# jinhan/tacotron2-vae

Measured on AMD Instinct MI355X. Metric: mel-frames/s (train step, batch=6, 80-mel), higher is better.
Workload: dtype f32; 1 GPU; configs[1]: Tacotron2-VAE fp32 train step (fwd+loss+bwd+clip+Adam), B=6/GPU fixed shape T_in=84 T_out=400, dropout on, random-init seed 1234; step_mode=hip-graph replay, decoder_forward=persistent, decoder_backward=persistent, startup_steps=43, global_batch=6, parallelism=dp1

## Files before the change

### include/t2vae.h

```cpp
#ifndef T2VAE_H
#define T2VAE_H
#include <stdint.h>
#ifdef __cplusplus
extern "C" {
#endif

#define T2V_OK 0
#define T2V_ERR_DIMS -1
#define T2V_ERR_ARG -2
#define T2V_ERR_LAUNCH -3

const char* t2v_version(void);
const char* t2v_last_error(void);

void t2v_set_phase_profile(unsigned long long* dev_buf32);
int t2v_stamp(unsigned long long* dev_buf, int slot, void* stream);
int t2v_debug_spin(int wgs, int microseconds, void* stream);

typedef struct t2v_step_params {
    uint64_t epoch;
    float lr;
    float bc1;
    float bc2s;
    float kl_weight;
// ... 210 lines not shown

int t2v_bn_act_fwd(const float* y, const float* stat_part, int nblk, const float* gamma, const float* beta,
                   float* running_mean, float* running_var, float* mean_out, float* rstd_out, float* out,
                   int B, int M, int T, int act, int training, float p_drop, float momentum, float eps,
                   uint64_t seed, uint32_t rng_stream, uint32_t rng_t, void* stream);
int t2v_bn_act_fwd_len(const float* y, const float* gamma, const float* beta, const float* running_mean,
                       const float* running_var, float* out, const int32_t* lengths, int B, int M, int T, int act, float eps,
                       void* stream);
int t2v_bn_act_bwd(const float* y, const float* dout, const float* mean, const float* rstd,
                   const float* gamma, const float* beta, float* dy, float* dgamma, float* dbeta,
                   float* dconv_bias, int B, int M, int T, int act, float p_drop, uint64_t seed,
                   uint32_t rng_stream, uint32_t rng_t, void* stream);
int t2v_bn_act_bwd_eval(const float* y, const float* dout, const float* mean, const float* rstd,
                   const float* gamma, const float* beta, float* dy, float* dgamma, float* dbeta,
                   float* dconv_bias, int B, int M, int T, int act, float p_drop, uint64_t seed,
                   uint32_t rng_stream, uint32_t rng_t, void* stream);

int t2v_embedding_fwd(const long long* ids, const float* W, float* out_bct, int B, int T, int C, int n_symbols, void* stream);
int t2v_embedding_bwd(const long long* ids, const float* dy_bct, float* dW, int B, int T, int C, int n_symbols, void* stream);

int t2v_gemm_epilogue_bwd(const float* dy, const float* y, float* out, size_t n, float scale, void* stream);

long t2v_colsum_scratch_floats(long M, long N);
int t2v_colsum(const float* A, long lda, long M, long N, float* scratch, float* out, void* stream);

int t2v_mask_outputs(float* mel, float* mel_post, float* gate, const int* lengths, int B, int C, int T, float gate_fill,
                     void* stream);
int t2v_mask_time(const float* x, float* out, const int32_t* lengths, int B, int C, int T, void* stream);
int t2v_reparam_fwd(const float* eps, const float* mu, const float* logvar, float* z, long n, void* stream);
int t2v_reparam_bwd(const float* dz, const float* eps, const float* logvar, float* dlogvar, long n, void* stream);
int t2v_gather_words(const void* const* src, void* const* dst, int n, void* stream);
int t2v_concat2_rows(const float* a, long lda, int na, const float* b, long ldb, int nb, float* out, long rows, void* stream);

int t2v_bilstm_fwd(const float* gx, const float* whh, const int32_t* lengths, float* y, float* gates,
                   float* cells, float* hx_scratch, uint32_t* sync3, int B, int T, void* stream);
int t2v_bilstm_bwd(const float* whh, const int32_t* lengths, const float* dy, const float* gates,
                   const float* cells, float* dg, float* dgx_scratch, uint32_t* sync3, int B, int T,
                   void* stream);

int t2v_gemm_f32(const float* A, long sAi, long sAk, const float* B, long sBj, long sBk, const float* bias,
                 float* C, int ldc, int M, int N, int K, int relu, int accumulate, float p_drop,
                 uint64_t seed, uint32_t rng_stream, uint32_t rng_t, void* stream);
long t2v_gemm_splitk_scratch_floats(int M, int N, int K);
int t2v_gemm_f32_splitk(const float* A, long sAi, long sAk, const float* B, long sBj, long sBk, const float* bias,
                        float* C, int ldc, int M, int N, int K, int relu, int accumulate, float p_drop,
                        uint64_t seed, uint32_t rng_stream, uint32_t rng_t, float* splitk_scratch, void* stream);

int t2v_gemm_f32_set_mode(int x3);

typedef struct t2v_gemm_group {
    const float* A;
    long sAi;
    long sAk;
    int nb;
    const float* B[3];
    long sBj[3];
    long sBk[3];
    int N[3];
    float* C[3];
    int ldc[3];
} t2v_gemm_group;
long t2v_gemm_f32_grouped_scratch_floats(const t2v_gemm_group* groups, int ngroups, int M, int K);
int t2v_gemm_f32_grouped(const t2v_gemm_group* groups, int ngroups, int M, int K, int accumulate, float* scratch, void* stream);
long t2v_gemm_f32_grouped_group_offset(const t2v_gemm_group* groups, int ngroups, int M, int K, int g);
int t2v_gemm_f32_grouped_handed(const t2v_gemm_group* groups, int ngroups, int M, int K, int accumulate, float* scratch, int handed,
                                const uint32_t* done_ctr, int done_cap, void* stream);
long t2v_gemm_bf16_grouped_scratch_floats(const t2v_gemm_group* groups, int ngroups, int M, int K);
int t2v_gemm_bf16_grouped(const t2v_gemm_group* groups, int ngroups, int M, int K, int accumulate, float* scratch, void* stream);
// ... 111 lines not shown
```

### tacotron2-vae_amd/csrc/bilstm.hip

```cpp
#include "t2v_common.h"
#include "t2v_kernels.h"
#include "t2v_coop.h"

#define BL_H 256
#define BL_G (4 * BL_H)
#define BL_NW 16
#define BL_UNITS (BL_H / BL_NW)
#define BL_NT (BL_UNITS / 16)

struct BiLstmFwdArgs {
    const float* gx;
    const float* whh;
    const int32_t* lengths;
    float* y;
    float* gates;
    float* cells;
    t2v_u64* hx;
    unsigned* sync;
    int B, T;
};

#define BL_SPIN 4000000u
__device__ __forceinline__ void bl_put(t2v_u64* p, float v, unsigned tag) {
    __hip_atomic_store(p, ((t2v_u64)tag << 32) | (t2v_u64)__float_as_uint(v), __ATOMIC_RELAXED, __HIP_MEMORY_SCOPE_AGENT);
}

template <int BQ>
__global__ __launch_bounds__(512) void k_bilstm_fwd(BiLstmFwdArgs a) {
    const int dir = blockIdx.x / BL_NW, j = blockIdx.x % BL_NW;
    const int tid = threadIdx.x, wave = (tid >> 6) & 3, kh = tid >> 8, lane = tid & 63;
    const int b = lane & 15, g = lane >> 4;
    const bool bvalid = b < a.B;
    __shared__ float hbuf[16][BL_H + 4];
    __shared__ f32x4 kpart[4][BL_NT][64];
    __shared__ int ok_flag;
    if (tid == 0) ok_flag = 1;
    float wreg[BL_NT][32];
    {
        const float* W = a.whh + (size_t)dir * BL_G * BL_H;
#pragma unroll
        for (int tt = 0; tt < BL_NT; ++tt) {
            const int unit = j * BL_UNITS + (BL_NT * wave + tt) * 4 + ((lane & 15) >> 2);
            const int row = (lane & 3) * BL_H + unit;
#pragma unroll
            for (int s = 0; s < 32; ++s) wreg[tt][s] = W[(size_t)row * BL_H + 4 * (32 * kh + s) + g];
        }
    }
    for (int i = tid; i < 16 * (BL_H + 4); i += 512) (&hbuf[0][0])[i] = 0.f;
    const int len = bvalid ? a.lengths[b] : 0;
    float cst[BL_NT];
#pragma unroll
    for (int tt = 0; tt < BL_NT; ++tt) cst[tt] = 0.f;
    __syncthreads();

    for (int step = 0; step < a.T; ++step) {
        const bool active = step < len;
        const int t = dir == 0 ? step : len - 1 - step;
        float gxv[BL_NT][4];
#pragma unroll
        for (int tt = 0; tt < BL_NT; ++tt) {
            const int U = j * BL_UNITS + (BL_NT * wave + tt) * 4 + g;
#pragma unroll
            for (int r = 0; r < 4; ++r)
                gxv[tt][r] = (active && kh == 0) ? a.gx[(((size_t)dir * a.B + b) * a.T + t) * BL_G + r * BL_H + U] : 0.f;
        }
        f32x4 accv[BL_NT];
#pragma unroll
        for (int tt = 0; tt < BL_NT; ++tt) accv[tt] = f32x4{0.f, 0.f, 0.f, 0.f};
        const float* hrow = &hbuf[b][g + 128 * kh];
#pragma unroll
        for (int s = 0; s < 32; ++s) {
            const float hv = hrow[4 * s];
#pragma unroll
            for (int tt = 0; tt < BL_NT; ++tt) accv[tt] = mfma16x4(wreg[tt][s], hv, accv[tt]);
        }
        if (kh == 1) {
#pragma unroll
            for (int tt = 0; tt < BL_NT; ++tt) kpart[wave][tt][lane] = accv[tt];
        }
        __syncthreads();
        if (kh == 0) {
#pragma unroll
            for (int tt = 0; tt < BL_NT; ++tt) accv[tt] += kpart[wave][tt][lane];
        }
        t2v_u64* hx_w = a.hx + ((size_t)(dir * 2 + (step & 1)) * 16) * BL_H;
#pragma unroll
        for (int tt = 0; tt < BL_NT; ++tt) {
            const f32x4 acc = accv[tt];
            const int U = j * BL_UNITS + (BL_NT * wave + tt) * 4 + g;
            if (bvalid && kh == 0) {
                float hnew = hbuf[b][U];
                float gi = 0.f, gf = 0.f, gg = 0.f, go = 0.f, c = 0.f;
                if (active) {
                    gi = sigmoidf_(acc[0] + gxv[tt][0]); gf = sigmoidf_(acc[1] + gxv[tt][1]);
                    gg = tanhf_(acc[2] + gxv[tt][2]); go = sigmoidf_(acc[3] + gxv[tt][3]);
                    c = gf * cst[tt] + gi * gg;
                    cst[tt] = c;
                    hnew = go * tanhf_(c);
                }
                bl_put(hx_w + (size_t)b * BL_H + U, hnew, (unsigned)step + 1u);
                if (active) {
                    a.y[((size_t)b * a.T + t) * (2 * BL_H) + dir * BL_H + U] = hnew;
                    if (a.gates) {
                        float* gs = a.gates + (((size_t)dir * a.B + b) * a.T + t) * BL_G + U;
                        gs[0] = gi; gs[BL_H] = gf; gs[2 * BL_H] = gg; gs[3 * BL_H] = go;
                        a.cells[(((size_t)dir * a.B + b) * a.T + t) * BL_H + U] = c;
                    }
                }
            }
        }
        if (step + 1 == a.T) break;
        {
            float hv[BQ];
            unsigned spins = 0;
            for (; tid < BL_H;) {
                bool ok = true;
#pragma unroll
                for (int u = 0; u < BQ; ++u) {
                    const t2v_u64 x = __hip_atomic_load(hx_w + (size_t)min(u, a.B - 1) * BL_H + tid, __ATOMIC_RELAXED, __HIP_MEMORY_SCOPE_AGENT);
                    hv[u] = __uint_as_float((unsigned)x);
                    ok = ok && (unsigned)(x >> 32) == (unsigned)step + 1u;
                }
                if (ok) break;
                __builtin_amdgcn_s_sleep(1);
                if (++spins > BL_SPIN || __hip_atomic_load(a.sync + 2, __ATOMIC_RELAXED, __HIP_MEMORY_SCOPE_AGENT)) {
                    __hip_atomic_store(a.sync + 2, 1u, __ATOMIC_RELAXED, __HIP_MEMORY_SCOPE_AGENT);
                    ok_flag = 0;
                    break;
                }
            }
            __syncthreads();
#pragma unroll
            for (int u = 0; u < BQ; ++u)
                if (u < a.B && tid < BL_H) hbuf[u][tid] = hv[u];
        }
        __syncthreads();
        if (!ok_flag) return;
    }
}

struct BiLstmBwdArgs {
    const float* whh;
    const int32_t* lengths;
    const float* dy;
    const float* gates;
    const float* cells;
    float* dg;
    t2v_u64* dgx;
    unsigned* sync;
    int B, T;
};

#define BLB_GR ((size_t)16 * 16 * BL_H)
__global__ __launch_bounds__(512) void k_bilstm_bwd(BiLstmBwdArgs a) {
    const int dir = blockIdx.x / BL_NW, j = blockIdx.x % BL_NW;
    const int tid = threadIdx.x, wave = tid >> 6, lane = tid & 63;
    const int b = lane & 15, g = lane >> 4;
    __shared__ __attribute__((aligned(16))) float dgl[16][64 + 4];
    __shared__ int ok_flag;
    if (tid == 0) ok_flag = 1;
    float wreg[2][16];
    {
        const float* W = a.whh + (size_t)dir * BL_G * BL_H;
#pragma unroll
        for (int s = 0; s < 16; ++s) {
            const int k = 4 * s + g;
            const int row = (k >> 4) * BL_H + j * BL_UNITS + (k & 15);
// ... 68 lines not shown
        }
        if (live) { dgl[bb][uu] = di; dgl[bb][16 + uu] = df; dgl[bb][32 + uu] = dgg; dgl[bb][48 + uu] = dob; }
        __syncthreads();
        if (!ok_flag) return;
        if (step == 0) break;
        {
            float bop[16];
#pragma unroll
            for (int s = 0; s < 16; ++s) bop[s] = dgl[b][4 * s + g];
            __builtin_amdgcn_sched_barrier(0);
            f32x4 acc[2];
#pragma unroll
            for (int tt = 0; tt < 2; ++tt) acc[tt] = f32x4{0.f, 0.f, 0.f, 0.f};
#pragma unroll
            for (int s = 0; s < 16; ++s)
#pragma unroll
                for (int tt = 0; tt < 2; ++tt) acc[tt] = mfma16x4(wreg[tt][s], bop[s], acc[tt]);
            if (b < a.B) {
                t2v_u64* dst = a.dgx + (size_t)(dir * 2 + (step & 1)) * BLB_GR + ((size_t)j * 16 + b) * BL_H + 32 * wave + 4 * g;
#pragma unroll
                for (int tt = 0; tt < 2; ++tt)
#pragma unroll
                    for (int r = 0; r < 4; ++r) bl_put(dst + 16 * tt + r, acc[tt][r], tag);
            }
        }
        if (on) {
            float* o = a.dg + idx * BL_G + U;
            o[0] = di; o[BL_H] = df; o[2 * BL_H] = dgg; o[3 * BL_H] = dob;
        }
        __syncthreads();
    }
}

extern "C" int t2v_bilstm_fwd(const float* gx, const float* whh, const int32_t* lengths, float* y, float* gates,
                              float* cells, float* hx_scratch, uint32_t* sync3, int B, int T, void* stream_) {
    hipStream_t stream = (hipStream_t)stream_;
    if (!gx || !whh || !lengths || !y || !hx_scratch || !sync3 || B < 1 || B > 16 || T < 1) return T2V_ERR_ARG;
    if ((gates == nullptr) != (cells == nullptr)) return T2V_ERR_ARG;
    T2VZeroRegions z;
    z.add(sync3, 3 * sizeof(uint32_t));
    z.add(hx_scratch, sizeof(t2v_u64) * 2 * 2 * 16 * BL_H);
    z.add(y, sizeof(float) * (size_t)B * T * 2 * BL_H);
    t2v_zero_regions(z, stream);
    BiLstmFwdArgs a;
    a.gx = gx; a.whh = whh; a.lengths = lengths; a.y = y; a.gates = gates; a.cells = cells; a.hx = (t2v_u64*)hx_scratch;
    a.sync = sync3; a.B = B; a.T = T;
    if (B <= 4) k_bilstm_fwd<4><<<2 * BL_NW, 512, 0, stream>>>(a);
    else if (B <= 8) k_bilstm_fwd<8><<<2 * BL_NW, 512, 0, stream>>>(a);
    else if (B <= 12) k_bilstm_fwd<12><<<2 * BL_NW, 512, 0, stream>>>(a);
    else k_bilstm_fwd<16><<<2 * BL_NW, 512, 0, stream>>>(a);
    return t2v_check_launch();
}

extern "C" int t2v_bilstm_bwd(const float* whh, const int32_t* lengths, const float* dy, const float* gates,
                              const float* cells, float* dg, float* dgx_scratch, uint32_t* sync3, int B, int T,
                              void* stream_) {
    hipStream_t stream = (hipStream_t)stream_;
    if (!whh || !lengths || !dy || !gates || !cells || !dg || !dgx_scratch || !sync3 || B < 1 || B > 16 || T < 1)
        return T2V_ERR_ARG;
    T2VZeroRegions z;
    z.add(sync3, 3 * sizeof(uint32_t));
    z.add(dgx_scratch, sizeof(t2v_u64) * 2 * 2 * BLB_GR);
    z.add(dg, sizeof(float) * (size_t)2 * B * T * BL_G);
    t2v_zero_regions(z, stream);
    BiLstmBwdArgs a;
    a.whh = whh; a.lengths = lengths; a.dy = dy; a.gates = gates; a.cells = cells; a.dg = dg; a.dgx = (t2v_u64*)dgx_scratch;
    a.sync = sync3; a.B = B; a.T = T;
    k_bilstm_bwd<<<2 * BL_NW, 512, 0, stream>>>(a);
    return t2v_check_launch();
}
```

### tacotron2-vae_amd/model.py

```python
from math import sqrt

import os

import torch
from torch import nn
from torch.nn import functional as F

import t2v_hip
from layers import ConvNorm, LinearNorm
from modules import VAE_GST
from utils import get_mask_from_lengths, to_gpu

drop_rate = 0.5
_drop_seed = [0x5EED]


class LocationLayer(nn.Module):
    def __init__(self, attention_n_filters, attention_kernel_size, attention_dim):
        super().__init__()
        self.location_conv = ConvNorm(2, attention_n_filters, kernel_size=attention_kernel_size,
                                      padding=(attention_kernel_size - 1) // 2, bias=False, stride=1,
                                      dilation=1)
        self.location_dense = LinearNorm(attention_n_filters, attention_dim, bias=False, w_init_gain='tanh')

# ... 509 lines not shown
            if mel.is_cuda and mel.is_contiguous() and mel_post.is_contiguous() and gate.is_contiguous():
                t2v_hip.mask_outputs(mel, mel_post, gate, lengths_i32(output_lengths, mel.device))
            else:
                pad = ~get_mask_from_lengths(output_lengths, outputs[0].size(2))
                mel.masked_fill_(pad.unsqueeze(1), 0.0)
                mel_post.masked_fill_(pad.unsqueeze(1), 0.0)
                gate.masked_fill_(pad, 1e3)
        return outputs

    def forward(self, inputs):
        with t2v_hip.defer_bn_counters():
            return self._forward(inputs)

    def _forward(self, inputs):
        text, input_lengths, targets, _, output_lengths, speakers, emotions = self.parse_input(inputs)
        if t2v_hip.step_params(create=False) is not None:
            _block_calls[0] = 0
            self.decoder._calls = 0
            if not self.training:
                self._eval_seq = (getattr(self, '_eval_seq', 0) + 1) % 4096
                _block_calls[0] = self._eval_seq * 64
                self.decoder._calls = self._eval_seq * 64
        ov = t2v_hip.overlap()
        if ov is not None:
            ov.on = bool(self.overlap_branches) and targets.is_cuda and os.environ.get('T2V_OVERLAP', '1') != '0'
        self.decoder.__dict__['_tf_t'] = (1 << 20) + _block_calls[0]
        fork = t2v_hip.mark()
        enc_first = os.environ.get('T2V_FWD_ORDER', 'enc_first') == 'enc_first' and fork is not None
        t2v_hip.BiLSTM._prep.clear()
        with t2v_hip.side('w', after=fork) as forked_p:
            if forked_p:
                l = self.encoder.lstm
                t2v_hip.BiLSTM.prepare(l.weight_hh_l0, l.bias_ih_l0, l.bias_hh_l0, l.weight_hh_l0_reverse, l.bias_ih_l0_reverse,
                                       l.bias_hh_l0_reverse)
        if enc_first:
            embedded = self.transcript_embedding(text).transpose(1, 2)
            transcript = self.encoder(embedded, input_lengths)
        with t2v_hip.side('vae', keep=(targets,), after=fork) as forked:
            style, mu, logvar, z = self.vae_gst(targets)
            t2v_hip.stamp('vae_fwd_end')
        with t2v_hip.side('w', keep=(targets,), after=fork) as forked_w:
            if forked_w:
                if self.training and torch.is_grad_enabled():
                    t2v_hip.preflip_conv_weights([blk[0].conv.weight for blk in self.encoder.convolutions]
                                                 + [blk[0].conv.weight for blk in self.postnet.convolutions])
                self.decoder.prepare(targets)
                t2v_hip.stamp('prenet_gpre_end')
        if not enc_first:
            embedded = self.transcript_embedding(text).transpose(1, 2)
            transcript = self.encoder(embedded, input_lengths)
        t2v_hip.stamp('encoder_end')
        if forked:
            ov.wait('vae')
            main = torch.cuda.current_stream()
            for t in (style, mu, logvar, z):
                t.record_stream(main)
        memory = transcript + style.unsqueeze(1)
        mel, gate, alignments = self.decoder(memory, targets, memory_lengths=input_lengths)
        mel_post = mel + self.postnet(mel)
        t2v_hip.stamp('postnet_fwd_end')
        return self.parse_output([mel, mel_post, gate, alignments, mu, logvar, z, emotions], output_lengths)
```

### tacotron2-vae_amd/t2v_hip.py

```python
import collections
import ctypes as C
import math
import os

import torch

_HERE = os.path.dirname(os.path.abspath(__file__))
_LIB_PATH = os.environ.get('T2V_LIB') or os.path.join(_HERE, 'libt2vae_hip.so')
_lib = None

H, E, PRE, A, F_LOC, KS, XW, KATT, KATT_INF, G4 = 1024, 512, 256, 128, 32, 31, 2560, 1536, 1792, 4096


class T2VHipError(RuntimeError):
    pass


class _DecWeights(C.Structure):
    _fields_ = [(n, C.c_void_p) for n in (
        'packF_att', 'packF_dec', 'packB_att', 'packB_dec', 'bias_att', 'bias_dec', 'wqT', 'wcomb', 'v')] + [
        ('packs_bf16', C.c_int32)]


class _DecTrainBufs(C.Structure):
# ... 18 lines not shown


class _DecTrainPersistWeights(C.Structure):
    C_NAME = 't2v_dec_train_persist_weights'
    _fields_ = [(n, C.c_void_p) for n in (
        'w_ih_att', 'w_hh_att', 'w_ih_dec', 'w_hh_dec', 'bias_dec', 'wq', 'wcomb', 'v')]


class _GemmGroup(C.Structure):
    C_NAME = 't2v_gemm_group'
    _fields_ = [('A', C.c_void_p), ('sAi', C.c_long), ('sAk', C.c_long), ('nb', C.c_int), ('B', C.c_void_p * 3), ('sBj', C.c_long * 3),
                ('sBk', C.c_long * 3), ('N', C.c_int * 3), ('C', C.c_void_p * 3), ('ldc', C.c_int * 3)]


class _AchainDw(C.Structure):
    C_NAME = 't2v_achain_dw'
    _fields_ = [('planes', C.c_void_p), ('d_w_ih', C.c_void_p), ('ld_ih', C.c_int), ('d_w_hh', C.c_void_p), ('ld_hh', C.c_int),
                ('accumulate', C.c_int), ('tile_cap', C.c_int)]


class _DecInferBufs(C.Structure):
    _fields_ = [(n, C.c_void_p) for n in (
        'memory', 'pm', 'lengths', 'XS', 'CA', 'CD', 'QP', 'AL', 'ACUM', 'PRE', 'MEL', 'GATE', 'stop_flag',
        'prenet_w1', 'proj_w', 'proj_b')]


class _DecItems(C.Structure):
    C_NAME = 't2v_dec_items'
    _fields_ = [(n, C.c_void_p) for n in ('stop_item', 'item_seeds')]


EXPORTS = ('t2v_version', 't2v_last_error', 't2v_stamp', 't2v_debug_spin', 't2v_pack_lstm_weights', 't2v_pack_lstm_weights_bf16', 't2v_decoder_train_fwd',
           't2v_decoder_train_bwd', 't2v_clip_adam_step', 't2v_clip_adam_step_guarded', 't2v_decoder_replay_fwd_kernels', 't2v_mel_frontend', 't2v_set_phase_profile', 't2v_decoder_infer_steps', 't2v_conv1d_stat_blocks', 't2v_conv1d_stat_blocks_bf16', 't2v_conv1d_fwd', 't2v_conv1d_bwd', 't2v_conv1d_fwd_bf16', 't2v_conv1d_bwd_bf16', 't2v_conv1d_dw_scratch_floats', 't2v_conv1d_flip_weights', 't2v_gemm_bf16', 't2v_gemm_bf16_splitk', 't2v_gemm_bf16_splitk_scratch_floats', 't2v_attn_wgrad', 't2v_attn_wgrad_scratch_floats',
           't2v_bn_act_fwd', 't2v_bn_act_bwd', 't2v_bn_act_bwd_eval', 't2v_bilstm_fwd', 't2v_bilstm_bwd', 't2v_gemm_f32', 't2v_conv2d_s2_fwd', 't2v_conv2d_s2_bwd', 't2v_conv2d_s2_dw_scratch_floats', 't2v_conv2d_s2_fwd_gemm', 't2v_conv2d_s2_bwd_gemm',
           't2v_conv2d_s2_gemm_scratch_floats',
           't2v_gru_fwd', 't2v_gru_bwd', 't2v_loss_fwd_bwd', 't2v_fuse_location_weights', 't2v_decoder_qp_floats',
           't2v_set_step_params', 't2v_set_step_params_stream', 't2v_decoder_replay_bwd_kernels', 't2v_embedding_fwd', 't2v_embedding_bwd', 't2v_gemm_f32_splitk', 't2v_gemm_splitk_scratch_floats', 't2v_gemm_f32_batched',
           't2v_decoder_infer_persistent', 't2v_decoder_persist_supported', 't2v_decoder_persist_scratch_floats',
           't2v_attn_bwd_slices', 't2v_colsum', 't2v_colsum_scratch_floats', 't2v_gemm_epilogue_bwd',
           't2v_decoder_train_fwd_persistent', 't2v_decoder_train_persist_supported',
           't2v_decoder_train_persist_scratch_floats', 't2v_decoder_bwd_persist_supported',
           't2v_decoder_bwd_achain_scratch_floats', 't2v_decoder_bwd_achain', 't2v_decoder_bwd_achain_prepare',
           't2v_decoder_bwd_achain_prepared', 't2v_decoder_bwd_persist_slices', 't2v_decoder_bwd_achain_dq_offset',
           't2v_decoder_bwd_achain_dw_offset', 't2v_gemm_f32_grouped_handed', 't2v_gemm_f32_grouped_group_offset', 't2v_mask_outputs', 't2v_reparam_fwd',
           't2v_reparam_bwd', 't2v_gather_words', 't2v_concat2_rows',
           't2v_decoder_train_fwd_persistent16', 't2v_decoder_train_persist16_supported',
           't2v_decoder_train_persist16_scratch_floats', 't2v_decoder_bwd_persistent16', 't2v_decoder_bwd_persist16_supported',
           't2v_decoder_bwd_persist16_scratch_floats', 't2v_decoder_bwd_persist16_dq_offset', 't2v_decoder_bwd_persist16_slices',
           't2v_decoder_bwd_persist16_fits', 't2v_gemm_f32_set_mode', 't2v_conv1d_x3_set_mode', 't2v_gemm_f32_grouped',
           't2v_gemm_f32_grouped_scratch_floats', 't2v_gemm_bf16_grouped', 't2v_gemm_bf16_grouped_scratch_floats',
           't2v_decoder_bwd_persistent16_prepare', 't2v_decoder_bwd_persistent16_prepared',
           't2v_stft_polar', 't2v_istft', 't2v_istft_scratch_bytes', 't2v_griffin_lim', 't2v_griffin_lim_scratch_bytes',
           't2v_mel_to_magnitude', 't2v_decoder_infer_steps_items', 't2v_decoder_infer_persistent_items', 't2v_bn_act_fwd_len',
           't2v_mask_time', 't2v_conv2d_s2_fwd_ragged', 't2v_conv2d_s2_fwd_gemm_ragged', 't2v_conv2d_s2_gemm_ragged_scratch_floats',
           't2v_gru_fwd_len', 't2v_mel_dtw', 't2v_mel_dtw_scratch_bytes', 't2v_tsne_scratch_bytes', 't2v_tsne_affinities',
           't2v_tsne_gradient', 't2v_tsne_run', 't2v_f0_yin', 't2v_alignment_stats', 't2v_alignment_scratch_bytes',
           't2v_mel_to_magnitude_nnls', 't2v_griffin_lim_fast', 't2v_griffin_lim_fast_scratch_bytes')


def lib_path():
    return _LIB_PATH


def load_library():
    global _lib
    if _lib is not None:
        return _lib
# ... 114 lines not shown
    lib.t2v_mel_to_magnitude_nnls.argtypes = [vp] * 7 + [C.c_float, C.c_int, vp, C.c_int, C.c_int, C.c_int, vp, vp]
    lib.t2v_griffin_lim_fast_scratch_bytes.argtypes = [C.c_int, C.c_int]
    lib.t2v_griffin_lim_fast_scratch_bytes.restype = C.c_size_t
    lib.t2v_griffin_lim_fast.argtypes = [vp, vp, vp, C.c_int, C.c_int, C.c_int, C.c_int, C.c_int, C.c_float, vp, vp, vp, vp,
                                         vp, C.c_int, vp]
    lib.t2v_mel_dtw_scratch_bytes.argtypes = [C.c_int, C.c_int, C.c_int]
    lib.t2v_mel_dtw_scratch_bytes.restype = C.c_size_t
    lib.t2v_mel_dtw.argtypes = [vp, vp, C.c_int, vp, vp, C.c_int, C.c_int, C.c_int, vp, vp, vp]
    lib.t2v_tsne_scratch_bytes.argtypes = [C.c_int, C.c_int]
    lib.t2v_tsne_scratch_bytes.restype = C.c_size_t
    lib.t2v_tsne_affinities.argtypes = [vp, C.c_int, C.c_int, C.c_float, vp, vp, vp]
    lib.t2v_tsne_gradient.argtypes = [vp, vp, C.c_int, C.c_float, vp, vp, vp, vp]
    lib.t2v_tsne_run.argtypes = [vp, vp, C.c_int, C.c_int, C.c_float, vp, vp, vp]
    lib.t2v_f0_yin.argtypes = [vp, vp, C.c_int, C.c_int, C.c_int, C.c_int, C.c_float, vp, vp, C.c_int, vp]
    lib.t2v_alignment_scratch_bytes.argtypes = [C.c_int, C.c_int, C.c_int]
    lib.t2v_alignment_scratch_bytes.restype = C.c_size_t
    lib.t2v_alignment_stats.argtypes = [vp, C.c_longlong, C.c_longlong, vp, vp, C.c_int, C.c_int, C.c_int, C.c_int, C.c_float, vp,
                                        C.c_int, vp, C.c_int, vp, vp, vp, vp]
    lib.t2v_conv1d_stat_blocks.argtypes = [C.c_int, C.c_int, C.c_int, C.c_int, C.c_int]
    lib.t2v_conv1d_stat_blocks_bf16.argtypes = [C.c_int, C.c_int, C.c_int, C.c_int, C.c_int]
    lib.t2v_conv1d_fwd.argtypes = [vp, vp, vp, vp, vp, C.c_int, C.c_int, C.c_int, C.c_int, C.c_int, vp]
    lib.t2v_conv1d_bwd.argtypes = [vp, vp, vp, vp, vp, vp, vp, C.c_int, C.c_int, C.c_int, C.c_int, C.c_int, vp]
    lib.t2v_conv1d_dw_scratch_floats.argtypes = [C.c_int] * 5
    lib.t2v_conv1d_flip_weights.argtypes = [vp, vp, vp, vp, C.c_int, C.c_int, vp]
    lib.t2v_conv1d_fwd_bf16.argtypes = [vp, vp, vp, vp, vp, vp, C.c_int, C.c_int, C.c_int, C.c_int, C.c_int, vp]
    lib.t2v_conv1d_bwd_bf16.argtypes = [vp, vp, vp, vp, vp, vp, vp, C.c_int, C.c_int, C.c_int, C.c_int, C.c_int, vp]
    lib.t2v_bn_act_fwd.argtypes = [vp, vp, C.c_int, vp, vp, vp, vp, vp, vp, vp, C.c_int, C.c_int, C.c_int, C.c_int,
                                   C.c_int, C.c_float, C.c_float, C.c_float, C.c_uint64, C.c_uint32, C.c_uint32, vp]
    lib.t2v_bn_act_bwd.argtypes = [vp, vp, vp, vp, vp, vp, vp, vp, vp, vp, C.c_int, C.c_int, C.c_int, C.c_int, C.c_float,
                                   C.c_uint64, C.c_uint32, C.c_uint32, vp]
    lib.t2v_bn_act_bwd_eval.argtypes = lib.t2v_bn_act_bwd.argtypes
    lib.t2v_bn_act_fwd_len.argtypes = [vp, vp, vp, vp, vp, vp, vp, C.c_int, C.c_int, C.c_int, C.c_int, C.c_float, vp]
    lib.t2v_mask_time.argtypes = [vp, vp, vp, C.c_int, C.c_int, C.c_int, vp]
    lib.t2v_bilstm_fwd.argtypes = [vp, vp, vp, vp, vp, vp, vp, vp, C.c_int, C.c_int, vp]
    lib.t2v_bilstm_bwd.argtypes = [vp, vp, vp, vp, vp, vp, vp, vp, C.c_int, C.c_int, vp]
    lib.t2v_gemm_f32.argtypes = [vp, C.c_long, C.c_long, vp, C.c_long, C.c_long, vp, vp, C.c_int, C.c_int, C.c_int,
                                 C.c_int, C.c_int, C.c_int, C.c_float, C.c_uint64, C.c_uint32, C.c_uint32, vp]
    lib.t2v_gemm_bf16.argtypes = lib.t2v_gemm_f32.argtypes
    lib.t2v_gemm_bf16_splitk.argtypes = lib.t2v_gemm_f32.argtypes[:-1] + [vp, vp]
    lib.t2v_gemm_bf16_splitk_scratch_floats.argtypes = [C.c_int, C.c_int, C.c_int]
    lib.t2v_gemm_bf16_splitk_scratch_floats.restype = C.c_long
    lib.t2v_gemm_f32_splitk.argtypes = lib.t2v_gemm_f32.argtypes[:-1] + [vp, vp]
    lib.t2v_gemm_f32_batched.argtypes = [vp, C.c_long, C.c_long, C.c_long, vp, C.c_long, C.c_long, C.c_long, vp, C.c_long,
                                         C.c_int, C.c_int, C.c_int, C.c_int, C.c_int, vp]
    lib.t2v_gemm_splitk_scratch_floats.argtypes = [C.c_int, C.c_int, C.c_int]
    lib.t2v_gemm_splitk_scratch_floats.restype = C.c_long
    lib.t2v_attn_wgrad.argtypes = [vp, vp, vp, vp, vp, vp, vp, vp, C.c_int, C.c_int, C.c_int, vp]
    lib.t2v_attn_wgrad_scratch_floats.argtypes = []
    lib.t2v_conv2d_s2_fwd.argtypes = [vp, vp, vp, vp, C.c_int, C.c_int, C.c_int, C.c_int, C.c_int, C.c_int, vp]
    lib.t2v_conv2d_s2_bwd.argtypes = [vp, vp, vp, vp, vp, vp, C.c_int, C.c_int, C.c_int, C.c_int, C.c_int, C.c_int, vp]
    lib.t2v_conv2d_s2_fwd_gemm.argtypes = [vp, vp, vp, vp, vp, C.c_int, C.c_int, C.c_int, C.c_int, C.c_int, C.c_int, vp]
    lib.t2v_conv2d_s2_bwd_gemm.argtypes = [vp, vp, vp, vp, vp, vp, C.c_int, C.c_int, C.c_int, C.c_int, C.c_int, C.c_int, vp]
    lib.t2v_conv2d_s2_gemm_scratch_floats.argtypes = [C.c_int] * 6
    lib.t2v_conv2d_s2_gemm_scratch_floats.restype = C.c_long
    lib.t2v_conv2d_s2_dw_scratch_floats.argtypes = [C.c_int] * 6
    lib.t2v_gru_fwd.argtypes = [vp, vp, vp, vp, vp, vp, vp, C.c_int, C.c_int, vp]
    lib.t2v_gru_bwd.argtypes = [vp, vp, vp, vp, vp, vp, vp, vp, C.c_int, C.c_int, vp]
    lib.t2v_conv2d_s2_fwd_ragged.argtypes = [vp, vp, vp, vp, vp] + [C.c_int] * 7 + [vp]
    lib.t2v_conv2d_s2_fwd_gemm_ragged.argtypes = [vp, vp, vp, vp, vp, vp] + [C.c_int] * 7 + [vp]
    lib.t2v_conv2d_s2_gemm_ragged_scratch_floats.argtypes = [C.c_int] * 6
    lib.t2v_conv2d_s2_gemm_ragged_scratch_floats.restype = C.c_long
    lib.t2v_gru_fwd_len.argtypes = [vp, vp, vp, vp, vp, vp, vp, vp, vp, C.c_int, C.c_int, vp]
    lib.t2v_loss_fwd_bwd.argtypes = [vp] * 15 + [C.c_uint64, C.c_int, C.c_int, C.c_float, vp]
    for name in EXPORTS:
        getattr(lib, name)
    _lib = lib
    return lib
# ... 1615 lines not shown
    else:
        _check(lib.t2v_conv1d_fwd(_p(w), _p(x), _p(bias), _p(y), None, B, Cin, T, Cout, KS, _stream()), 't2v_conv1d_fwd')
    out = torch.empty_like(y)
    _check(lib.t2v_bn_act_fwd_len(_p(y), _p(gamma), _p(beta), _p(running_mean), _p(running_var), _p(out), _p(lengths_i32),
                                  B, Cout, T, int(act), 1e-5, _stream()), 't2v_bn_act_fwd_len')
    return out


class Reparam(torch.autograd.Function):

    @staticmethod
    def forward(ctx, eps, mu, logvar):
        lib = _require_gpu(eps, mu, logvar)
        eps, mu, logvar = _f32c(eps), _f32c(mu), _f32c(logvar)
        z = torch.empty_like(mu)
        _check(lib.t2v_reparam_fwd(_p(eps), _p(mu), _p(logvar), _p(z), mu.numel(), _stream()), 't2v_reparam_fwd')
        ctx.save_for_backward(eps, logvar)
        return z

    @staticmethod
    def backward(ctx, dz):
        eps, logvar = ctx.saved_tensors
        dz = _f32c(dz)
        dlv = torch.empty_like(logvar)
        _check(load_library().t2v_reparam_bwd(_p(dz), _p(eps), _p(logvar), _p(dlv), dz.numel(), _stream()), 't2v_reparam_bwd')
        return None, dz, dlv


class BiLSTM(torch.autograd.Function):

    _prep = {}

    @staticmethod
    def prepare(w_hh, b_ih, b_hh, w_hh_r, b_ih_r, b_hh_r):
        with torch.no_grad():
            whh = torch.stack((w_hh, w_hh_r)).contiguous()
            bias, bias_r = b_ih + b_hh, b_ih_r + b_hh_r
        ev = torch.cuda.Event()
        ev.record()
        BiLSTM._prep[id(w_hh)] = (whh, bias, bias_r, ev)

    @staticmethod
    def forward(ctx, x, lengths, w_ih, w_hh, b_ih, b_hh, w_ih_r, w_hh_r, b_ih_r, b_hh_r, save):
        lib = _require_gpu(x, w_ih)
        B, T, _ = x.shape
        f32 = dict(device=x.device, dtype=torch.float32)
        x = _f32c(x)
        prep = BiLSTM._prep.pop(id(w_hh), None)
        if prep is not None:
            whh, bias, bias_r, ev = prep
            cur = torch.cuda.current_stream()
            cur.wait_event(ev)
            for t in (whh, bias, bias_r):
                t.record_stream(cur)
        else:
            whh = torch.stack((w_hh, w_hh_r)).contiguous()
            bias, bias_r = b_ih + b_hh, b_ih_r + b_hh_r
        y = torch.empty(B, T, 512, **f32)
        chunks = []
        for b0 in range(0, B, MAX_DEC_B):
            b1 = min(B, b0 + MAX_DEC_B)
            Bc = b1 - b0
            gx = torch.empty(2, Bc, T, 1024, **f32)
            gemm(x[b0:b1].view(Bc * T, -1), w_ih, bias, out=gx[0].view(Bc * T, 1024))
            gemm(x[b0:b1].view(Bc * T, -1), w_ih_r, bias_r, out=gx[1].view(Bc * T, 1024))
            gates = torch.empty(2, Bc, T, 1024, **f32) if save else None
            cells = torch.empty(2, Bc, T, 256, **f32) if save else None
            hx = torch.empty(2 * 2 * 2 * 16 * 256, **f32)
            sync = torch.empty(3, device=x.device, dtype=torch.int32)
            _check(lib.t2v_bilstm_fwd(_p(gx), _p(whh), _p(lengths[b0:b1]), _p(y[b0:b1]), _p(gates), _p(cells), _p(hx),
                                      _p(sync), Bc, T, _stream()), 't2v_bilstm_fwd')
            _err_note('BiLSTM forward', sync[2:3])
            chunks.append((b0, b1, gates, cells, sync))
        ctx.keep = (x, lengths, w_ih, w_ih_r, whh, y.detach(), chunks)
        ctx.dims = (B, T)
        return y

    @staticmethod
    def backward(ctx, dy):
        lib = load_library()
        x, lengths, w_ih, w_ih_r, whh, y, chunks = ctx.keep
        B, T = ctx.dims
        if chunks[0][2] is None:
            raise T2VHipError("BiLSTM forward ran without saving activations")
        f32 = dict(device=x.device, dtype=torch.float32)
        dy = _f32c(dy)
        dg = torch.empty(2, B, T, 1024, **f32) if len(chunks) == 1 else None
        dgs = []
        stamp('bilstm_bwd_begin')
        for b0, b1, gates, cells, sync in chunks:
            Bc = b1 - b0
            dg_c = dg if dg is not None else torch.empty(2, Bc, T, 1024, **f32)
            dgx = torch.empty(2 * 2 * 2 * 16 * 16 * 256, **f32)
            _check(lib.t2v_bilstm_bwd(_p(whh), _p(lengths[b0:b1]), _p(dy[b0:b1]), _p(gates), _p(cells), _p(dg_c), _p(dgx),
                                      _p(sync), Bc, T, _stream()), 't2v_bilstm_bwd')
            _err_note('BiLSTM backward', sync[2:3])
            dgs.append(dg_c)
        stamp('bilstm_bwd_end')
        BT = B * T
        if dg is None:
            dg = torch.cat(dgs, 1)
        d0, d1, x2 = dg[0].reshape(BT, 1024), dg[1].reshape(BT, 1024), x.view(BT, -1)
        fork = mark()
        dx = gemm(d0, w_ih.t())
# ... 379 lines not shown
```

Before: 228,300 mel-frames/s.

## Replace tagged 64-bit hx exchange with sentinel-filled per-step rows in BiLSTM forward

The BiLSTM forward kernel used to exchange the hidden state through a double-buffered ring of 64-bit tagged words polled one scalar at a time. It now writes each step's hidden state to its own row of a sentinel-prefilled buffer sized T*B*H. Consumers poll with 16-byte vector buffer loads until no sentinel remains, so the tag traffic and per-element atomics go away. The sentinel fill can be done ahead of time on a forked side stream via prepare(), which moves that cost off the critical path. The trade-off is a larger scratch buffer and an extra fill kernel.

New measurement: 228,000 mel-frames/s. About the same (-0.1%).

```diff
diff --git a/include/t2vae.h b/include/t2vae.h
--- a/include/t2vae.h
+++ b/include/t2vae.h
@@ -266,8 +266,10 @@
 int t2v_gather_words(const void* const* src, void* const* dst, int n, void* stream);
 int t2v_concat2_rows(const float* a, long lda, int na, const float* b, long ldb, int nb, float* out, long rows, void* stream);
 
+long t2v_bilstm_hx_floats(int B, int T);
+int t2v_bilstm_fill(float* hx_rows, int B, int T, void* stream);
 int t2v_bilstm_fwd(const float* gx, const float* whh, const int32_t* lengths, float* y, float* gates,
-                   float* cells, float* hx_scratch, uint32_t* sync3, int B, int T, void* stream);
+                   float* cells, float* hx_rows, uint32_t* sync3, int B, int T, int hx_filled, void* stream);
 int t2v_bilstm_bwd(const float* whh, const int32_t* lengths, const float* dy, const float* gates,
                    const float* cells, float* dg, float* dgx_scratch, uint32_t* sync3, int B, int T,
                    void* stream);
diff --git a/tacotron2-vae_amd/csrc/bilstm.hip b/tacotron2-vae_amd/csrc/bilstm.hip
--- a/tacotron2-vae_amd/csrc/bilstm.hip
+++ b/tacotron2-vae_amd/csrc/bilstm.hip
@@ -1,6 +1,7 @@
 #include "t2v_common.h"
 #include "t2v_kernels.h"
 #include "t2v_coop.h"
+#include "t2v_xchg.h"
 
 #define BL_H 256
 #define BL_G (4 * BL_H)
@@ -15,7 +16,7 @@
     float* y;
     float* gates;
     float* cells;
-    t2v_u64* hx;
+    float* hx;
     unsigned* sync;
     int B, T;
 };
@@ -25,13 +26,12 @@
     __hip_atomic_store(p, ((t2v_u64)tag << 32) | (t2v_u64)__float_as_uint(v), __ATOMIC_RELAXED, __HIP_MEMORY_SCOPE_AGENT);
 }
 
-template <int BQ>
 __global__ __launch_bounds__(512) void k_bilstm_fwd(BiLstmFwdArgs a) {
     const int dir = blockIdx.x / BL_NW, j = blockIdx.x % BL_NW;
     const int tid = threadIdx.x, wave = (tid >> 6) & 3, kh = tid >> 8, lane = tid & 63;
     const int b = lane & 15, g = lane >> 4;
     const bool bvalid = b < a.B;
-    __shared__ float hbuf[16][BL_H + 4];
+    __shared__ __attribute__((aligned(16))) float hbuf[16][BL_H + 4];
     __shared__ f32x4 kpart[4][BL_NT][64];
     __shared__ int ok_flag;
     if (tid == 0) ok_flag = 1;
@@ -48,6 +48,11 @@
     }
     for (int i = tid; i < 16 * (BL_H + 4); i += 512) (&hbuf[0][0])[i] = 0.f;
     const int len = bvalid ? a.lengths[b] : 0;
+    const int pitem = ((tid >> 6) + 4) & 7;
+    int plen[2];
+#pragma unroll
+    for (int q = 0; q < 2; ++q) plen[q] = pitem + 8 * q < a.B ? a.lengths[pitem + 8 * q] : 0;
+    const __amdgpu_buffer_rsrc_t rx = t2v_rsrc(a.hx + (size_t)dir * a.T * a.B * BL_H);
     float cst[BL_NT];
 #pragma unroll
     for (int tt = 0; tt < BL_NT; ++tt) cst[tt] = 0.f;
@@ -56,6 +61,7 @@
     for (int step = 0; step < a.T; ++step) {
         const bool active = step < len;
         const int t = dir == 0 ? step : len - 1 - step;
+        const unsigned row = (unsigned)(step * a.B) * (unsigned)(BL_H * 4);
         float gxv[BL_NT][4];
 #pragma unroll
         for (int tt = 0; tt < BL_NT; ++tt) {
@@ -83,56 +89,40 @@
 #pragma unroll
             for (int tt = 0; tt < BL_NT; ++tt) accv[tt] += kpart[wave][tt][lane];
         }
-        t2v_u64* hx_w = a.hx + ((size_t)(dir * 2 + (step & 1)) * 16) * BL_H;
 #pragma unroll
         for (int tt = 0; tt < BL_NT; ++tt) {
             const f32x4 acc = accv[tt];
             const int U = j * BL_UNITS + (BL_NT * wave + tt) * 4 + g;
-            if (bvalid && kh == 0) {
-                float hnew = hbuf[b][U];
-                float gi = 0.f, gf = 0.f, gg = 0.f, go = 0.f, c = 0.f;
-                if (active) {
-                    gi = sigmoidf_(acc[0] + gxv[tt][0]); gf = sigmoidf_(acc[1] + gxv[tt][1]);
-                    gg = tanhf_(acc[2] + gxv[tt][2]); go = sigmoidf_(acc[3] + gxv[tt][3]);
-                    c = gf * cst[tt] + gi * gg;
-                    cst[tt] = c;
-                    hnew = go * tanhf_(c);
+            if (active && kh == 0) {
+                const float gi = sigmoidf_(acc[0] + gxv[tt][0]), gf = sigmoidf_(acc[1] + gxv[tt][1]);
+                const float gg = tanhf_(acc[2] + gxv[tt][2]), go = sigmoidf_(acc[3] + gxv[tt][3]);
+                const float c = gf * cst[tt] + gi * gg;
+                cst[tt] = c;
+                const float hnew = go * tanhf_(c);
+                if (step + 1 < len) t2v_st(rx, row + (unsigned)(b * BL_H + U) * 4u, hnew);
+                a.y[((size_t)b * a.T + t) * (2 * BL_H) + dir * BL_H + U] = hnew;
+                if (a.gates) {
+                    float* gs = a.gates + (((size_t)dir * a.B + b) * a.T + t) * BL_G + U;
+                    gs[0] = gi; gs[BL_H] = gf; gs[2 * BL_H] = gg; gs[3 * BL_H] = go;
+                    a.cells[(((size_t)dir * a.B + b) * a.T + t) * BL_H + U] = c;
                 }
-                bl_put(hx_w + (size_t)b * BL_H + U, hnew, (unsigned)step + 1u);
-                if (active) {
-                    a.y[((size_t)b * a.T + t) * (2 * BL_H) + dir * BL_H + U] = hnew;
-                    if (a.gates) {
-                        float* gs = a.gates + (((size_t)dir * a.B + b) * a.T + t) * BL_G + U;
-                        gs[0] = gi; gs[BL_H] = gf; gs[2 * BL_H] = gg; gs[3 * BL_H] = go;
-                        a.cells[(((size_t)dir * a.B + b) * a.T + t) * BL_H + U] = c;
-                    }
-                }
             }
         }
         if (step + 1 == a.T) break;
-        {
-            float hv[BQ];
-            unsigned spins = 0;
-            for (; tid < BL_H;) {
-                bool ok = true;
-#pragma unroll
-                for (int u = 0; u < BQ; ++u) {
-                    const t2v_u64 x = __hip_atomic_load(hx_w + (size_t)min(u, a.B - 1) * BL_H + tid, __ATOMIC_RELAXED, __HIP_MEMORY_SCOPE_AGENT);
-                    hv[u] = __uint_as_float((unsigned)x);
-                    ok = ok && (unsigned)(x >> 32) == (unsigned)step + 1u;
-                }
-                if (ok) break;
+#pragma unroll
+        for (int q = 0; q < 2; ++q) {
+            if (step + 1 >= plen[q]) continue;
+            const int item = pitem + 8 * q;
+            const unsigned off = row + (unsigned)(item * BL_H + 4 * lane) * 4u;
+            f32x4 v;
+            unsigned spins = 0, fails = 0;
+            for (;;) {
+                v = t2v_ld_f32x4(rx, off);
+                if (__all(t2v_ok4(v))) break;
                 __builtin_amdgcn_s_sleep(1);
-                if (++spins > BL_SPIN || __hip_atomic_load(a.sync + 2, __ATOMIC_RELAXED, __HIP_MEMORY_SCOPE_AGENT)) {
-                    __hip_atomic_store(a.sync + 2, 1u, __ATOMIC_RELAXED, __HIP_MEMORY_SCOPE_AGENT);
-                    ok_flag = 0;
-                    break;
-                }
-            }
-            __syncthreads();
-#pragma unroll
-            for (int u = 0; u < BQ; ++u)
-                if (u < a.B && tid < BL_H) hbuf[u][tid] = hv[u];
+                if ((++fails & 15u) == 0u && t2v_give_up(spins, BL_SPIN / 16u, a.sync + 2, &ok_flag)) break;
+            }
+            *(f32x4*)&hbuf[item][4 * lane] = v;
         }
         __syncthreads();
         if (!ok_flag) return;
@@ -267,23 +257,35 @@
     }
 }
 
+extern "C" long t2v_bilstm_hx_floats(int B, int T) {
+    return B < 1 || T < 1 ? 0 : (long)2 * T * B * BL_H;
+}
+
+extern "C" int t2v_bilstm_fill(float* hx_rows, int B, int T, void* stream_) {
+    if (!hx_rows || ((uintptr_t)hx_rows & 15) || B < 1 || B > 16 || T < 1 || (size_t)T * B * BL_H * 4 >= 0x7fffffffu) return T2V_ERR_ARG;
+    const size_t n16 = (size_t)t2v_bilstm_hx_floats(B, T) / 4;
+    const size_t grid = (n16 + 255) / 256;
+    t2v_fill_sentinel(hx_rows, n16, (int)(grid > 1024 ? 1024 : grid), (hipStream_t)stream_);
+    return t2v_check_launch();
+}
+
 extern "C" int t2v_bilstm_fwd(const float* gx, const float* whh, const int32_t* lengths, float* y, float* gates,
-                              float* cells, float* hx_scratch, uint32_t* sync3, int B, int T, void* stream_) {
+                              float* cells, float* hx_rows, uint32_t* sync3, int B, int T, int hx_filled, void* stream_) {
     hipStream_t stream = (hipStream_t)stream_;
-    if (!gx || !whh || !lengths || !y || !hx_scratch || !sync3 || B < 1 || B > 16 || T < 1) return T2V_ERR_ARG;
+    if (!gx || !whh || !lengths || !y || !hx_rows || !sync3 || B < 1 || B > 16 || T < 1) return T2V_ERR_ARG;
     if ((gates == nullptr) != (cells == nullptr)) return T2V_ERR_ARG;
+    if (!hx_filled) {
+        const int rc = t2v_bilstm_fill(hx_rows, B, T, stream_);
+        if (rc != T2V_OK) return rc;
+    } else if (((uintptr_t)hx_rows & 15) || (size_t)T * B * BL_H * 4 >= 0x7fffffffu) return T2V_ERR_ARG;
     T2VZeroRegions z;
     z.add(sync3, 3 * sizeof(uint32_t));
-    z.add(hx_scratch, sizeof(t2v_u64) * 2 * 2 * 16 * BL_H);
     z.add(y, sizeof(float) * (size_t)B * T * 2 * BL_H);
     t2v_zero_regions(z, stream);
     BiLstmFwdArgs a;
-    a.gx = gx; a.whh = whh; a.lengths = lengths; a.y = y; a.gates = gates; a.cells = cells; a.hx = (t2v_u64*)hx_scratch;
+    a.gx = gx; a.whh = whh; a.lengths = lengths; a.y = y; a.gates = gates; a.cells = cells; a.hx = hx_rows;
     a.sync = sync3; a.B = B; a.T = T;
-    if (B <= 4) k_bilstm_fwd<4><<<2 * BL_NW, 512, 0, stream>>>(a);
-    else if (B <= 8) k_bilstm_fwd<8><<<2 * BL_NW, 512, 0, stream>>>(a);
-    else if (B <= 12) k_bilstm_fwd<12><<<2 * BL_NW, 512, 0, stream>>>(a);
-    else k_bilstm_fwd<16><<<2 * BL_NW, 512, 0, stream>>>(a);
+    k_bilstm_fwd<<<2 * BL_NW, 512, 0, stream>>>(a);
     return t2v_check_launch();
 }
 
diff --git a/tacotron2-vae_amd/model.py b/tacotron2-vae_amd/model.py
--- a/tacotron2-vae_amd/model.py
+++ b/tacotron2-vae_amd/model.py
@@ -565,7 +565,7 @@
             if forked_p:
                 l = self.encoder.lstm
                 t2v_hip.BiLSTM.prepare(l.weight_hh_l0, l.bias_ih_l0, l.bias_hh_l0, l.weight_hh_l0_reverse, l.bias_ih_l0_reverse,
-                                       l.bias_hh_l0_reverse)
+                                       l.bias_hh_l0_reverse, shape=tuple(text.shape[:2]))
         if enc_first:
             embedded = self.transcript_embedding(text).transpose(1, 2)
             transcript = self.encoder(embedded, input_lengths)
diff --git a/tacotron2-vae_amd/t2v_hip.py b/tacotron2-vae_amd/t2v_hip.py
--- a/tacotron2-vae_amd/t2v_hip.py
+++ b/tacotron2-vae_amd/t2v_hip.py
@@ -74,7 +74,7 @@
 
 EXPORTS = ('t2v_version', 't2v_last_error', 't2v_stamp', 't2v_debug_spin', 't2v_pack_lstm_weights', 't2v_pack_lstm_weights_bf16', 't2v_decoder_train_fwd',
            't2v_decoder_train_bwd', 't2v_clip_adam_step', 't2v_clip_adam_step_guarded', 't2v_decoder_replay_fwd_kernels', 't2v_mel_frontend', 't2v_set_phase_profile', 't2v_decoder_infer_steps', 't2v_conv1d_stat_blocks', 't2v_conv1d_stat_blocks_bf16', 't2v_conv1d_fwd', 't2v_conv1d_bwd', 't2v_conv1d_fwd_bf16', 't2v_conv1d_bwd_bf16', 't2v_conv1d_dw_scratch_floats', 't2v_conv1d_flip_weights', 't2v_gemm_bf16', 't2v_gemm_bf16_splitk', 't2v_gemm_bf16_splitk_scratch_floats', 't2v_attn_wgrad', 't2v_attn_wgrad_scratch_floats',
-           't2v_bn_act_fwd', 't2v_bn_act_bwd', 't2v_bn_act_bwd_eval', 't2v_bilstm_fwd', 't2v_bilstm_bwd', 't2v_gemm_f32', 't2v_conv2d_s2_fwd', 't2v_conv2d_s2_bwd', 't2v_conv2d_s2_dw_scratch_floats', 't2v_conv2d_s2_fwd_gemm', 't2v_conv2d_s2_bwd_gemm',
+           't2v_bn_act_fwd', 't2v_bn_act_bwd', 't2v_bn_act_bwd_eval', 't2v_bilstm_fwd', 't2v_bilstm_bwd', 't2v_bilstm_fill', 't2v_bilstm_hx_floats', 't2v_gemm_f32', 't2v_conv2d_s2_fwd', 't2v_conv2d_s2_bwd', 't2v_conv2d_s2_dw_scratch_floats', 't2v_conv2d_s2_fwd_gemm', 't2v_conv2d_s2_bwd_gemm',
            't2v_conv2d_s2_gemm_scratch_floats',
            't2v_gru_fwd', 't2v_gru_bwd', 't2v_loss_fwd_bwd', 't2v_fuse_location_weights', 't2v_decoder_qp_floats',
            't2v_set_step_params', 't2v_set_step_params_stream', 't2v_decoder_replay_bwd_kernels', 't2v_embedding_fwd', 't2v_embedding_bwd', 't2v_gemm_f32_splitk', 't2v_gemm_splitk_scratch_floats', 't2v_gemm_f32_batched',
@@ -255,7 +255,10 @@
     lib.t2v_bn_act_bwd_eval.argtypes = lib.t2v_bn_act_bwd.argtypes
     lib.t2v_bn_act_fwd_len.argtypes = [vp, vp, vp, vp, vp, vp, vp, C.c_int, C.c_int, C.c_int, C.c_int, C.c_float, vp]
     lib.t2v_mask_time.argtypes = [vp, vp, vp, C.c_int, C.c_int, C.c_int, vp]
-    lib.t2v_bilstm_fwd.argtypes = [vp, vp, vp, vp, vp, vp, vp, vp, C.c_int, C.c_int, vp]
+    lib.t2v_bilstm_fwd.argtypes = [vp, vp, vp, vp, vp, vp, vp, vp, C.c_int, C.c_int, C.c_int, vp]
+    lib.t2v_bilstm_fill.argtypes = [vp, C.c_int, C.c_int, vp]
+    lib.t2v_bilstm_hx_floats.argtypes = [C.c_int, C.c_int]
+    lib.t2v_bilstm_hx_floats.restype = C.c_long
     lib.t2v_bilstm_bwd.argtypes = [vp, vp, vp, vp, vp, vp, vp, vp, C.c_int, C.c_int, vp]
     lib.t2v_gemm_f32.argtypes = [vp, C.c_long, C.c_long, vp, C.c_long, C.c_long, vp, vp, C.c_int, C.c_int, C.c_int,
                                  C.c_int, C.c_int, C.c_int, C.c_float, C.c_uint64, C.c_uint32, C.c_uint32, vp]
@@ -1937,13 +1940,29 @@
     _prep = {}
 
     @staticmethod
-    def prepare(w_hh, b_ih, b_hh, w_hh_r, b_ih_r, b_hh_r):
+    def _chunks(B):
+        return [(b0, min(B, b0 + MAX_DEC_B)) for b0 in range(0, B, MAX_DEC_B)]
+
+    @staticmethod
+    def _rows(Bc, T, device, fill):
+        lib = load_library()
+        hx = torch.empty(lib.t2v_bilstm_hx_floats(Bc, T), device=device, dtype=torch.float32)
+        if fill:
+            _check(lib.t2v_bilstm_fill(_p(hx), Bc, T, _stream()), 't2v_bilstm_fill')
+        return hx
+
+    @staticmethod
+    def prepare(w_hh, b_ih, b_hh, w_hh_r, b_ih_r, b_hh_r, shape=None):
         with torch.no_grad():
             whh = torch.stack((w_hh, w_hh_r)).contiguous()
             bias, bias_r = b_ih + b_hh, b_ih_r + b_hh_r
+        rows = None
+        if shape is not None:
+            B, T = shape
+            rows = (B, T, [BiLSTM._rows(b1 - b0, T, w_hh.device, True) for b0, b1 in BiLSTM._chunks(B)])
         ev = torch.cuda.Event()
         ev.record()
-        BiLSTM._prep[id(w_hh)] = (whh, bias, bias_r, ev)
+        BiLSTM._prep[id(w_hh)] = (whh, bias, bias_r, rows, ev)
 
     @staticmethod
     def forward(ctx, x, lengths, w_ih, w_hh, b_ih, b_hh, w_ih_r, w_hh_r, b_ih_r, b_hh_r, save):
@@ -1952,29 +1971,31 @@
         f32 = dict(device=x.device, dtype=torch.float32)
         x = _f32c(x)
         prep = BiLSTM._prep.pop(id(w_hh), None)
+        rows = None
         if prep is not None:
-            whh, bias, bias_r, ev = prep
+            whh, bias, bias_r, rows, ev = prep
             cur = torch.cuda.current_stream()
             cur.wait_event(ev)
-            for t in (whh, bias, bias_r):
+            if rows is not None and rows[:2] != (B, T):
+                rows = None
+            for t in (whh, bias, bias_r) + (tuple(rows[2]) if rows is not None else ()):
                 t.record_stream(cur)
         else:
             whh = torch.stack((w_hh, w_hh_r)).contiguous()
             bias, bias_r = b_ih + b_hh, b_ih_r + b_hh_r
         y = torch.empty(B, T, 512, **f32)
         chunks = []
-        for b0 in range(0, B, MAX_DEC_B):
-            b1 = min(B, b0 + MAX_DEC_B)
+        for ci, (b0, b1) in enumerate(BiLSTM._chunks(B)):
             Bc = b1 - b0
             gx = torch.empty(2, Bc, T, 1024, **f32)
             gemm(x[b0:b1].view(Bc * T, -1), w_ih, bias, out=gx[0].view(Bc * T, 1024))
             gemm(x[b0:b1].view(Bc * T, -1), w_ih_r, bias_r, out=gx[1].view(Bc * T, 1024))
             gates = torch.empty(2, Bc, T, 1024, **f32) if save else None
             cells = torch.empty(2, Bc, T, 256, **f32) if save else None
-            hx = torch.empty(2 * 2 * 2 * 16 * 256, **f32)
+            hx = rows[2][ci] if rows is not None else BiLSTM._rows(Bc, T, x.device, False)
             sync = torch.empty(3, device=x.device, dtype=torch.int32)
             _check(lib.t2v_bilstm_fwd(_p(gx), _p(whh), _p(lengths[b0:b1]), _p(y[b0:b1]), _p(gates), _p(cells), _p(hx),
-                                      _p(sync), Bc, T, _stream()), 't2v_bilstm_fwd')
+                                      _p(sync), Bc, T, 1 if rows is not None else 0, _stream()), 't2v_bilstm_fwd')
             _err_note('BiLSTM forward', sync[2:3])
             chunks.append((b0, b1, gates, cells, sync))
         ctx.keep = (x, lengths, w_ih, w_ih_r, whh, y.detach(), chunks)
```
